# h3jia/bayesfast

Measured on AMD Instinct MI355X. Metric: leapfrog steps/sec (all chains), 4096 chains x 64-d quadratic surrogate, higher is better.
Workload: dtype f64

## Files before the change

bayesfast_amd/_lib.py:

```python
import ctypes as C
import os
import subprocess

_HERE = os.path.dirname(os.path.abspath(__file__))
LIB_PATH = os.environ.get('BFHIP_LIBRARY') or os.path.join(_HERE, 'libbfhip.so')
CSRC = os.path.join(_HERE, 'csrc')

SC_FIELDS = ('log_step', 'log_bar', 'hbar', 'mu', 'count', 'fg_n', 'bg_n', 'n_samples', 'prev_update',
             'adapt_window', 'i_iter', 'error')
SC_N = len(SC_FIELDS)
VEC_FIELDS = ('q', 'var', 'fg_mean', 'fg_raw', 'bg_mean', 'bg_raw')
VEC_N = len(VEC_FIELDS)
MAT_N = 6
STAT_STRIDE = 11
NSTATS = ('logp', 'energy', 'tree_depth', 'tree_size', 'mean_tree_accept', 'step_size', 'step_size_bar',
          'warmup', 'energy_change', 'max_energy_change', 'diverging')
HSTATS = ('logp', 'energy', 'n_int_step', 'accept_stat', 'accepted', 'step_size', 'step_size_bar', 'warmup',
          'energy_change', 'diverging')
MAX_DIM = 128
MAX_TREEDEPTH = 12
TREE_MODE_WORK = 4162
LAG_EDGES = tuple((j + 1) if j < 2 else ((1 << ((j + 1) // 2)) if (j & 1) else (3 << (j // 2 - 1))) for j in range(64))

_dp = C.POINTER(C.c_double)
# ... 49 lines not shown
    'bfhip_ctx_destroy': (None, [_vp]),
    'bfhip_ctx_set_stream': (C.c_int, [_vp, _vp]),
    'bfhip_ctx_synchronize': (C.c_int, [_vp]),
    'bfhip_density_upload': (C.c_int, [_vp, C.POINTER(DensityDesc)]),
    'bfhip_logp_grad': (C.c_int, [_vp, C.c_int, _vp, C.c_int, _vp, _vp]),
    'bfhip_constraint': (C.c_int, [_vp, C.c_int, C.c_int, _vp, _vp, _vp]),
    'bfhip_leapfrog': (C.c_int, [_vp, C.c_int] + [_vp] * 8),
    'bfhip_sampler_run': (C.c_int, [_vp, C.POINTER(SamplerConfig), C.c_int, C.c_int, _vp, _vp, _vp, C.c_int,
                                    C.c_int, _vp, _vp, _vp]),
    'bfhip_tnuts_run': (C.c_int, [_vp, C.POINTER(SamplerConfig), C.POINTER(Tempering), C.c_int, C.c_int, _vp, _vp, _vp, _vp,
                                  C.c_int, C.c_int, _vp, _vp, _vp, _vp]),
    'bfhip_rng_seed': (C.c_int, [_vp, C.c_int, C.c_uint64, C.c_uint64, _vp]),
    'bfhip_chain_init': (C.c_int, [_vp, C.c_int, C.c_int, _vp, C.c_double, _vp, _vp, C.c_double, C.c_int, _vp, _vp]),
    'bfhip_metric_init_full': (C.c_int, [_vp, C.c_int, C.c_int, _vp, C.c_double, _vp, _vp]),
    'bfhip_polymodel_upload': (C.c_int, [_vp, C.POINTER(PolymodelDesc)]),
    'bfhip_polymodel_eval': (C.c_int, [_vp, C.c_int, _vp, _vp, _vp]),
    'bfhip_chi2_stage': (C.c_int, [_vp, C.c_int, C.c_int, C.c_int, _vp, _vp, _vp, _vp, _vp, C.c_double, _vp, _vp]),
    'bfhip_pipeline_upload': (C.c_int, [_vp, C.POINTER(PipelineDesc)]),
    'bfhip_design_block': (C.c_int, [_vp, C.c_int, C.c_int, C.c_int, _vp, _vp, _vp, C.c_int, C.c_int]),
    'bfhip_gram': (C.c_int, [_vp, C.c_int, C.c_int, C.c_int, _vp, C.c_int, _vp, _vp, _vp]),
    'bfhip_tree_size_mode_share': (C.c_int, [_vp, C.c_int, C.c_int, _vp, C.c_int, C.c_int, C.c_double, _vp]),
    'bfhip_solve_spd': (C.c_int, [_vp, C.c_int, C.c_int, _vp, _vp, _vp]),
    'bfhip_lstsq': (C.c_int, [_vp, C.c_int, C.c_int, C.c_int, _vp, C.c_int, _vp, _vp, _vp, C.c_int, _vp, _vp]),
    'bfhip_sort_keys': (C.c_int, [_vp, C.c_long, _vp, _vp, _vp]),
    'bfhip_order_keys': (C.c_int, [_vp, C.c_long, _vp, _vp]),
    'bfhip_count_keys': (C.c_int, [_vp, C.c_long, _vp, C.c_long, _vp, C.c_int, _vp]),
    'bfhip_importance_weights': (C.c_int, [_vp, C.c_long, _vp, _vp, C.c_double, _vp, _vp]),
    'bfhip_polar_ns': (C.c_int, [_vp, C.c_int, _vp, _vp, C.c_int, _vp, _vp]),
    'bfhip_ndtri': (C.c_int, [_vp, C.c_long, _vp, _vp]),
    'bfhip_ica_tanh': (C.c_int, [_vp, C.c_long, C.c_long, C.c_int, _vp, _vp]),
    'bfhip_ica_assemble': (C.c_int, [_vp, C.c_int, C.c_int, _vp, C.c_long, C.c_long, _vp, _vp, _vp, _vp]),
    'bfhip_ica_post': (C.c_int, [_vp, C.c_int, _vp, _vp, _vp, C.c_int, C.c_int, _vp, _vp]),
    'bfhip_spline_build': (C.c_int, [_vp, C.c_int, C.c_long, _vp, _vp, _vp, _vp, C.c_int, _vp, C.c_int, C.c_int, _vp, C.c_double,
                                     C.c_int, C.c_int, C.c_int, _vp, _vp, _vp, _vp]),
    'bfhip_kde_cdf': (C.c_int, [_vp, C.c_int, C.c_long, _vp, _vp, _vp, C.c_int, _vp, _vp]),
    'bfhip_spline_apply': (C.c_int, [_vp, C.c_int, C.c_long, C.c_int, _vp, _vp, _vp, _vp, _vp, _vp]),
    'bfhip_bridge_sums': (C.c_int, [_vp, C.c_long, _vp, C.c_long, _vp, C.c_double, _vp]),
    'bfhip_bridge_terms': (C.c_int, [_vp, C.c_long, _vp, _vp, C.c_long, _vp, _vp, C.c_double, _vp, _vp]),
    'bfhip_logmeanexp_stats': (C.c_int, [_vp, C.c_long, _vp, _vp, _vp, _vp]),
    'bfhip_acor_moments': (C.c_int, [_vp, C.c_int, C.c_long, C.c_int, C.c_long, _vp, _vp, _vp]),
    'bfhip_acor_lag_sums': (C.c_int, [_vp, C.c_int, C.c_long, C.c_int, C.c_long, _vp, _vp, _vp, C.c_long, C.c_int, _vp, _vp]),
    'bfhip_diag_columns': (C.c_int, [_vp, C.c_int, C.c_long, C.c_long, C.c_long, _vp, C.c_int, C.c_long, C.c_int, C.c_int, C.c_int, _vp,
                                     _vp]),
    'bfhip_diag_extent': (C.c_int, [_vp, C.c_int, C.c_long, _vp, _vp, _vp]),
    'bfhip_diag_sort': (C.c_int, [_vp, C.c_long, _vp, C.c_int, _vp, _vp]),
    'bfhip_diag_rank': (C.c_int, [_vp, C.c_long, _vp, _vp, C.c_int, _vp]),
    'bfhip_logp_hess': (C.c_int, [_vp, C.c_int, _vp, C.c_int, _vp, _vp, _vp]),
    'bfhip_laplace_opt': (C.c_int, [_vp, C.POINTER(LaplaceOpts), C.c_int, _vp, _vp, _vp, _vp, _vp]),
    'bfhip_pipeline_logp_hess': (C.c_int, [_vp, C.c_int, _vp, C.c_int, C.c_int, _vp, _vp, _vp]),
    'bfhip_pipeline_laplace_opt': (C.c_int, [_vp, C.POINTER(LaplaceOpts), C.c_int, C.c_int, _vp, _vp, _vp, _vp, _vp]),
    'bfhip_wave_sum_probe': (C.c_int, [_vp, C.c_int, C.c_int, C.c_int, _vp, _vp]),
}
HESS_FULL, HESS_GAUSS_NEWTON = 0, 1
WSUM_MAX = 7
WSUM_FORMS = {'built': 0, 'packed': 1, 'unpacked': 2}
ACOR_MAX_GROUPS = 256
DIAG_BATCH = 16

_lib = None


def build(verbose=False):
    out = None if verbose else subprocess.DEVNULL
    subprocess.check_call(['make', '-C', CSRC, '-j4'], stdout=out)
    return LIB_PATH


def lib():
    global _lib
    if _lib is None:
        if not os.path.exists(LIB_PATH):
            raise RuntimeError(
                'bayesfast_amd: the HIP extension %s is missing; build it with '
                '`python -c "import __graft_entry__ as g; g.build()"` or `make -C bayesfast_amd/csrc`. '
                'There is no CPU fallback.' % LIB_PATH)
        import torch
        L = C.CDLL(LIB_PATH)
        for name, (res, args) in SYMBOLS.items():
            f = getattr(L, name)
            f.restype = res
            f.argtypes = args
        _lib = L
    return _lib


class BfhipError(RuntimeError):
    pass


def debug_set(key, value):
    f = lib().bfhip_debug_set
    f.restype, f.argtypes = C.c_int, [C.c_char_p, C.c_longlong]
    check(f(key.encode(), int(value)))


def debug_get(key):
    f = lib().bfhip_debug_get
    f.restype, f.argtypes = C.c_longlong, [C.c_char_p]
    return int(f(key.encode()))


def debug_buffer(key, tensor_or_none):
    f = lib().bfhip_debug_buffer
    f.restype, f.argtypes = C.c_int, [C.c_char_p, C.c_void_p]
    check(f(key.encode(), None if tensor_or_none is None else C.c_void_p(tensor_or_none.data_ptr())))


# ... 12 lines not shown
```

bayesfast_amd/csrc/bfhip_lone.h:

```cpp

#pragma push_macro("exp")
#pragma push_macro("log")
#pragma push_macro("sqrt")
#pragma push_macro("sincospi")
#undef exp
#undef log
#undef sqrt
#undef sincospi
__device__ inline double ln_opq(double x) { asm("" : "+v"(x)); return x; }
#define LN_EXPV(x) ln_opq(exp(ln_opq(x)))
#define LN_LOGV(x) ln_opq(log(ln_opq(x)))
#define LN_SQRTV(x) ln_opq(sqrt(ln_opq(x)))
#define LN_EXP(x) rfl(LN_EXPV(x))
#define LN_LOG(x) rfl(LN_LOGV(x))
#define LN_SQRT(x) rfl(LN_SQRTV(x))

enum { LN_CONT = 0, LN_NEW = 1, LN_DONE = 2 };
enum { LF_NONE = 0, LF_LEAF = 1, LF_INIT = 2 };
enum { LV_CMD = 0, LV_CLOSE, LV_EO, LV_EVAL, LV_DIR, LV_INIT, LV_N = 8 };

template <int W, int DEC>
struct LoneGeo {
    using PG = PipeGeo<W, DEC>;
    static constexpr int DP = 16 * W, NS = 4 * W, NMAT = PG::NMAT, KS = PG::KS, KPJ = PG::KPJ;
// ... 375 lines not shown
            WF[2 * DP + lane] = load_vec(BFHIP_VEC_BG_MEAN, 0.); WF[3 * DP + lane] = load_vec(BFHIP_VEC_BG_RAW, 0.);
        }
        if (lane < 5) WF[4 * DP + lane] = scp[BFHIP_SC_FG_N + lane];
    }
    if (i_iter < a.iter_end && err == 0) {
        draw_momentum();
        eps = (i_iter < nw) ? step_now : step_bar;
        draw_dir();
        post_new(1);
        fly = LF_INIT;
    } else {
        if (lane == 0) VI[LV_CMD] = LN_DONE;
        kdone = true;
    }

    for (;;) {
        LTRACE(1, 0);
        __syncthreads();
        LTRACE(1, 1);
        if (kdone) break;
        kb = 0;
        bool ended = false;
        if (prev == LF_INIT) {
            q = lfv(0); p = lfv(1); g = lfv(2);
            const double E0 = rfl(LF[3 * DP]), logp0 = rfl(LF[3 * DP + 1]);
            KBAR(); KBAR();
            if (!init_tree(E0, logp0)) { kdone = true; }
        } else if (prev == LF_LEAF) {
            {
                const double lq_ = lfv(0), lp_ = lfv(1), lg_ = lfv(2);
                const double le_ = LF[3 * DP], ll_ = LF[3 * DP + 1];
                TPq = lq_; TRp = lp_; TPg = lg_;
                E_pend = rfl(le_);
                lp_pend = rfl(ll_);
            }
            LTRACE(1, 4);
            int unit = U_EVAL, lev = 0;
            nlf += 1;
            n_prop += 1;
            double dE = E_pend - start_energy;
            if (dE != dE) dE = INFINITY;
            if (fabs(dE) > fabs(max_de)) max_de = dE;
            T_E = E_pend;
            T_logp = lp_pend;
            T_acc = 0.;
            if (!(fabs(dE) < a.cfg.max_change)) {
                diverged = 1;
                unit = U_ABORT;
            }
            LTRACE(1, 11);
            KBAR();
            LTRACE(1, 10);
            double aw = -dE - w_off;
            const double e_aw = LN_EXPV(aw);
            const double ps0 = L0p + TRp;
            double r2[2] = {ps0 * (var * L0p), ps0 * (var * TRp)};
            wave_sum_n<2>(r2);
            if (unit == U_EVAL) {
                T_W = rfl(e_aw);
                if (aw > 600.) {
                    const double sc_ = LN_EXP(-aw);
                    tree_W = tree_W * sc_;
                    if (lane == 0)
                        for (int l2 = 0; l2 < depth; ++l2) LS[l2 * LS_N + LS_LS] *= sc_;
                    L0_W *= sc_;
                    w_off = w_off + aw;
                    aw = 0.;
                    T_W = 1.;
                }
                const double pacc = (w_off == 0.) ? T_W : LN_EXP(-dE);
                T_acc = pacc > 1. ? 1. : pacc;
                TLp = TRp;
                TPs = TRp;
                unit = U_MERGE;
            }
            LTRACE(1, 5);
            if (unit == U_MERGE && (i_leaf & 1) && depth > 0) {
                T_acc = L0_acc + T_acc;
                const double Wsum = L0_W + T_W;
                if (Wsum != Wsum) err = 2;
                const double u = bf_u01(bf_xoshiro_next(rs));
                lev = 1;
                if ((r2[0] <= 0.) || (r2[1] <= 0.)) {
                    unit = U_ABORT;
                } else {
                    if (!((u * Wsum < T_W) || (u == 0.))) {
                        TPq = L0q;
                        TPg = L0g;
                        T_E = rfl(LS[LS_E]);
                        T_logp = rfl(LS[LS_LOGP]);
                    }
                    T_W = Wsum;
                    TPs = L0p + TRp;
                    TLp = L0p;
                }
            }
            LTRACE(1, 6);
            KBAR();
            LTRACE(1, 7);
            while (unit == U_MERGE && lev < depth && ((i_leaf >> lev) & 1)) {
                const int slot = SL_STACK + 4 * lev;
                const double A = ldv(slot + 0), B = ldv(slot + 1), S1 = ldv(slot + 2);
                const double psum = S1 + TPs;
                const double vA = var * A, vB = var * B, vC = var * TLp, vD = var * TRp;
                const double ps1 = S1 + TLp;
                const double ps2 = B + TPs;
                double r6[6] = {psum * vA, psum * vD, ps1 * vA, ps1 * vC, ps2 * vB, ps2 * vD};
                wave_sum_n<6>(r6);
                const bool turning = (r6[0] <= 0.) || (r6[1] <= 0.) || (r6[2] <= 0.) || (r6[3] <= 0.) || (r6[4] <= 0.) || (r6[5] <= 0.);
                const double *lsp = LS + lev * LS_N;
                T_acc = rfl(lsp[LS_ACC]) + T_acc;
                const double Wsum = rfl(lsp[LS_LS]) + T_W;
                if (Wsum != Wsum) err = 2;
                const double u = bf_u01(bf_xoshiro_next(rs));
                const bool keep_t2 = (u * Wsum < T_W) || (u == 0.);
                lev += 1;
                if (turning) {
                    unit = U_ABORT;
                } else {
                    if (!keep_t2) {
                        TPq = ldv(slot + 3);
                        TPg = ldv(SL_PG + lev - 1);
                        T_E = rfl(lsp[LS_E]);
                        T_logp = rfl(lsp[LS_LOGP]);
                    }
                    T_W = Wsum;
                    TLp = A;
                    TPs = psum;
                }
            }
            if (unit == U_MERGE) {
                if (lev < depth) {
                    if (lev == 0) {
                        L0p = TRp;
                        L0q = TPq;
                        L0g = TPg;
                        L0_W = T_W;
                        L0_acc = T_acc;
                    } else {
                        const int slot = SL_STACK + 4 * lev;
                        stv(slot + 0, TLp); stv(slot + 1, TRp); stv(slot + 2, TPs); stv(slot + 3, TPq);
                        stv(SL_PG + lev, TPg);
                    }
                    if (lane == 0) {
                        double *lsp = LS + lev * LS_N;
                        lsp[LS_LS] = T_W; lsp[LS_ACC] = T_acc;
                        lsp[LS_E] = (lev == 0) ? E_pend : T_E;
                        lsp[LS_LOGP] = (lev == 0) ? lp_pend : T_logp;
                    }
                    i_leaf += 1;
                    unit = U_DONE;
                } else {
                    unit = U_DBL_END;
                }
            }
            LTRACE(1, 8);
            if (unit == U_ABORT) {
                for (int al = (diverged ? 0 : lev); al < depth; ++al)
                    if ((i_leaf >> al) & 1) T_acc = rfl(LS[al * LS_N + LS_ACC]) + T_acc;
                depth += 1;
                acc_sum += T_acc;
                unit = U_END1;
            } else if (unit == U_DBL_END) {
                double ps = ldv(SL_PSUM);
                const double oldL = ldv(SL_LEFT_P), oldR = ldv(SL_RIGHT_P);
                depth += 1;
                acc_sum += T_acc;
                {
                    if (T_W != T_W || tree_W != tree_W) err = 2;
                    const double u = bf_u01(bf_xoshiro_next(rs));
                    if ((u * tree_W < T_W) || (u == 0.)) {
                        stv(SL_PROP_Q, TPq);
                        stv(SL_PROPG, TPg);
                        prop_E = T_E;
                        prop_logp = T_logp;
                    }
                    tree_W = tree_W + T_W;
                }
                ps += TPs;
                const double vN = var * TRp, vT = var * TLp, vL = var * oldL, vR = var * oldR;
                double r6[6];
                if (dir > 0) {
                    const double ps1 = ps + TLp, ps2 = oldR + TPs;
// ... 182 lines not shown
```

bayesfast_amd/csrc/bfhip_nuts_pipe.h:

```cpp


enum { SL_PROPG = SL_STACK + 4 * BFHIP_MAX_TREEDEPTH, SL_PG = SL_PROPG + 1, SL_PIPE_N = SL_PG + BFHIP_MAX_TREEDEPTH };

template <int W, int DEC = 0>
struct PipeGeo {
    static constexpr int NMAT = DEC == 1 ? 3 : 2;
    static constexpr int KS = DEC == 1 ? (W == 2 ? 2 : 1) : ((W == 2 || W == 4) ? 2 : 1);
    static constexpr int KPJ = (4 * W) / KS, NJOB = NMAT * W * KS, NTL = 12;
    static constexpr int MPS = KPJ > 8 ? 2 : 1;
    static_assert(NJOB <= 16 && KPJ <= 8 * MPS, "one job per wave, eight MFMA sites");
    static constexpr size_t lds_doubles() {
        using G = SamplerGeo<W>;
        return (size_t)NMAT * G::NS * G::XS + (size_t)16 * BFHIP_MAX_TREEDEPTH * LS_N + 4 + (size_t)16 * CS_N +
               (size_t)16 * NTL * G::DP + (size_t)NMAT * KS * 16 * G::GS;
    }
};

template <int QUAD> struct PipeAcc { typedef d4_t type; };
template <> struct PipeAcc<1> { typedef double type; };
template <> struct PipeAcc<2> { typedef d2_t type; };
__device__ inline d4_t bf_pipe_mfma(double a_, double b_, d4_t c_) { return __builtin_amdgcn_mfma_f64_16x16x4f64(a_, b_, c_, 0, 0, 0); }
__device__ inline double bf_pipe_mfma(double a_, double b_, double c_) { return __builtin_amdgcn_mfma_f64_4x4x4f64(a_, b_, c_, 0, 0, 0); }

template <int W, bool TR, int DEC = 0, int QUAD = 0>
__global__ __launch_bounds__(1024) void bf_nuts_pipe_kernel(DevModel m, SamplerArgs a) {
    using G = SamplerGeo<W>;
    using PG = PipeGeo<W, DEC>;
    constexpr int DP = G::DP, NS = G::NS, XS = G::XS, GS = G::GS;
    constexpr int KS_P = PG::KS, KPJ_P = PG::KPJ, NJOB_P = PG::NJOB, NTL = PG::NTL, NMAT = PG::NMAT, MPS = PG::MPS;
    constexpr int MAXL = BFHIP_MAX_TREEDEPTH;
    static_assert(DP <= 64, "one dimension per lane");
    extern __shared__ __attribute__((aligned(16))) double lds[];
    double *XB = lds;
    double *LS = XB + NMAT * NS * XS;
    int *alive = (int *)(LS + 16 * MAXL * LS_N);
    double *CS = LS + 16 * MAXL * LS_N + 4;
    double *TB = CS + 16 * CS_N;
    double *GB = TB + 16 * NTL * DP;

    const int tid = threadIdx.x, lane = tid & 63;
    const int w = __builtin_amdgcn_readfirstlane(tid >> 6);
    int cpg = a.cpg > 0 ? a.cpg : 16;
    int chain = blockIdx.x * cpg + w;
    bool real = w < cpg && chain < a.n_chain;
    if (a.tail_list) {
        const int cnt = rfl(a.tail_count[0]);
        cpg = cnt <= a.n_cu ? 1 : (cnt <= 2 * a.n_cu ? 2 : 4);
        const int idx = blockIdx.x * cpg + w;
        real = w < cpg && idx < cnt;
        chain = real ? rfl(a.tail_list[idx]) : 0;
    }
    const int d = m.d;
    const bool lane_ok = lane < DP;

    double afr[KPJ_P];
    {
        const int slot_m = w / (W * KS_P), rem = w % (W * KS_P), t = rem / KS_P, kp = rem % KS_P;
        const double *Af = (slot_m == 0 ? m.Sf : (slot_m == 1 ? m.Hf : m.Hdf)) + (t * NS + kp * KPJ_P) * 64 + lane;
#pragma unroll
        for (int s = 0; s < KPJ_P; ++s) afr[s] = (w < NJOB_P) ? Af[s * 64] : 0.;
    }
    if (tid < 8) alive[tid] = 0;
    const double c_lin = lane_ok ? m.pd[PD_LIN * DP + lane] : 0.;
    const double c_mu = lane_ok ? m.pd[PD_MU * DP + lane] : 0.;
    const double c_dmu = (DEC == 1 && lane_ok) ? m.pd[PD_DMU * DP + lane] : 0.;
    const double c_smu = lane_ok ? m.pd[PD_SMU * DP + lane] : 0.;
    const int c_kind = (TR && lane_ok) ? (int)m.pd[PD_KIND * DP + lane] : 0;
    const double c_lo = (TR && lane_ok) ? m.pd[PD_LO * DP + lane] : 0., c_rg = (TR && lane_ok) ? m.pd[PD_RG * DP + lane] : 1.;
    double xs = 0., jac = 1., gj = 0., logdet_l = 0.;

    double q = 0., p = 0., g = 0., var = 1.;
    double TLp = 0., TPs = 0., TPq = 0.;
    double TRp = 0.;
    double L0p = 0., L0q = 0.;
    double TPg = 0., L0g = 0.;
    uint64_t rs[4] = {0, 0, 0, 0};
    int i_iter = 0, mode = M_DONE, err = 0;
    double eps = 0., eps_t = 0.;
    int dir = 1, depth = 0, i_leaf = 0, n_prop = 0, diverged = 0;
    double start_energy = 0., acc_sum = 0.;
    double T_W = 0., T_acc = 0.;
    double max_de = 0., w_off = 0., L0_W = 0., L0_acc = 0.;
    bool pend = false;
// ... 242 lines not shown
                const int xi = (lane >> 2) * XS + w + 16 * (lane & 3);
                XB[xi] = xs;
                XB[NS * XS + xi] = xs - c_mu;
                if constexpr (DEC == 1) XB[2 * NS * XS + xi] = xs - c_dmu;
            }
        }
        if (lane == 0) {
            if (mode != M_DONE) alive[trip & 1] = 1;
            if (evaluating) atomicOr((unsigned *)&alive[2 + (trip & 1)], 1u << w);
        }
        TRACE(1);
        __syncthreads();
        TRACE(2);
        if (rfl(alive[trip & 1]) == 0) break;
        const unsigned ev_mask = (unsigned)rfl(alive[2 + (trip & 1)]);
        if (tid == 0) { alive[(trip + 1) & 1] = 0; alive[2 + ((trip + 1) & 1)] = 0; alive[4 + ((trip + 1) & 1)] = 0; }

        const bool job = ev_mask != 0 && w < NJOB_P;
        typename PipeAcc<QUAD>::type acc = {};
        const double *Xf = XB + ((w / (W * KS_P)) * NS + (w % KS_P) * KPJ_P) * XS + (QUAD ? (lane & ~15) + (lane & 3) : lane);
        double x_pre[MPS], x_pr2[QUAD == 2 ? MPS : 1];
#pragma unroll
        for (int u = 0; u < MPS; ++u) x_pre[u] = job ? Xf[u * XS] : 0.;
        if constexpr (QUAD == 2) {
#pragma unroll
            for (int u = 0; u < MPS; ++u) x_pr2[u] = job ? Xf[u * XS + 4] : 0.;
        }
#define BF_MF(K)                                                                                            \
        do {                                                                                                \
            if ((K) * MPS < KPJ_P) {                                                                        \
                double x_cur[MPS], x_cu2[QUAD == 2 ? MPS : 1];                                             \
                _Pragma("unroll") for (int u = 0; u < MPS; ++u) x_cur[u] = x_pre[u];                        \
                if constexpr (QUAD == 2) { _Pragma("unroll") for (int u = 0; u < MPS; ++u) x_cu2[u] = x_pr2[u]; } \
                if (((K) + 1) * MPS < KPJ_P && job) {                                                       \
                    _Pragma("unroll") for (int u = 0; u < MPS; ++u) x_pre[u] = Xf[((((K) + 1) * MPS < KPJ_P ? ((K) + 1) * MPS : 0) + u) * XS]; \
                    if constexpr (QUAD == 2) { _Pragma("unroll") for (int u = 0; u < MPS; ++u) x_pr2[u] = Xf[((((K) + 1) * MPS < KPJ_P ? ((K) + 1) * MPS : 0) + u) * XS + 4]; } \
                }                                                                                           \
                _Pragma("unroll") for (int u = 0; u < MPS; ++u) {                                           \
                    asm volatile("" : "+v"(acc) : : "memory");                                              \
                    if constexpr (QUAD == 2) {                                                              \
                        if (job) {                                                                          \
                            acc[0] = bf_pipe_mfma(afr[((K) * MPS < KPJ_P ? (K) * MPS : 0) + u], x_cur[u], acc[0]); \
                            acc[1] = bf_pipe_mfma(afr[((K) * MPS < KPJ_P ? (K) * MPS : 0) + u], x_cu2[u], acc[1]); \
                        }                                                                                   \
                    } else {                                                                                \
                        if (job) acc = bf_pipe_mfma(afr[((K) * MPS < KPJ_P ? (K) * MPS : 0) + u], x_cur[u], acc); \
                    }                                                                                       \
                    asm volatile("" : "+v"(acc) : : "memory");                                              \
                }                                                                                           \
            }                                                                                               \
        } while (0)
        int unit = pend ? U_EVAL : U_DONE, lev = 0;
        bool ended = false;
        pend = false;
        BF_MF(0);
        TRACE(3);
        double dE = 0.;
        if (unit == U_EVAL) {
            nlf += 1;
            n_prop += 1;
            dE = E_pend - start_energy;
            if (dE != dE) dE = INFINITY;
            if (fabs(dE) > fabs(max_de)) max_de = dE;
            cs_set(CS_T_E, E_pend);
            cs_set(CS_T_LOGP, lp_pend);
            T_acc = 0.;
            if (!(fabs(dE) < a.cfg.max_change)) {
                diverged = 1;
                unit = U_ABORT;
            }
        }
        BF_MF(1);
        if (unit == U_EVAL) {
            double aw = -dE - w_off;
            if (aw > 600.) {
                const double sc_ = uexp(-aw);
                cs_set(CS_TREE_W, cs_get(CS_TREE_W) * sc_);
                if (lane == 0)
                    for (int l2 = 0; l2 < depth; ++l2) lsw[l2 * LS_N + LS_LS] *= sc_;
                L0_W *= sc_;
                w_off = w_off + aw;
                aw = 0.;
            }
            T_W = uexp(aw);
            const double pacc = (w_off == 0.) ? T_W : uexp(-dE);
            T_acc = pacc > 1. ? 1. : pacc;
            TLp = TRp;
            TPs = TRp;
            unit = U_MERGE;
        }
        BF_MF(2);
        TRACE(9);
        if (unit == U_MERGE && (i_leaf & 1) && depth > 0) {
            const double ps0 = L0p + TRp;
            double r2[2] = {ps0 * (var * L0p), ps0 * (var * TRp)};
            wave_sum_n<2>(r2);
            T_acc = L0_acc + T_acc;
            const double Wsum = L0_W + T_W;
            if (Wsum != Wsum) err = 2;
            const double u = bf_u01(bf_xoshiro_next(rs));
            lev = 1;
            if ((r2[0] <= 0.) || (r2[1] <= 0.)) {
                unit = U_ABORT;
            } else {
                if (!((u * Wsum < T_W) || (u == 0.))) {
                    TPq = L0q;
                    TPg = L0g;
                    cs_set(CS_T_E, rfl(lsw[LS_E]));
                    cs_set(CS_T_LOGP, rfl(lsw[LS_LOGP]));
                }
                T_W = Wsum;
                TPs = L0p + TRp;
                TLp = L0p;
            }
        }
        BF_MF(3);
        while (unit == U_MERGE && lev < depth && ((i_leaf >> lev) & 1)) {
            const int slot = SL_STACK + 4 * lev;
            const double A = ldv(slot + 0), B = ldv(slot + 1), S1 = ldv(slot + 2);
            const double psum = S1 + TPs;
            const double vA = var * A, vB = var * B, vC = var * TLp, vD = var * TRp;
            const double ps1 = S1 + TLp;
            const double ps2 = B + TPs;
            double r6[6] = {psum * vA, psum * vD, ps1 * vA, ps1 * vC, ps2 * vB, ps2 * vD};
            wave_sum_n<6>(r6);
            const bool turning = (r6[0] <= 0.) || (r6[1] <= 0.) || (r6[2] <= 0.) || (r6[3] <= 0.) || (r6[4] <= 0.) || (r6[5] <= 0.);
            const double *lsp = lsw + lev * LS_N;
            T_acc = rfl(lsp[LS_ACC]) + T_acc;
            const double Wsum = rfl(lsp[LS_LS]) + T_W;
            if (Wsum != Wsum) err = 2;
            const double u = bf_u01(bf_xoshiro_next(rs));
            const bool keep_t2 = (u * Wsum < T_W) || (u == 0.);
            lev += 1;
            if (turning) {
                unit = U_ABORT;
            } else {
                if (!keep_t2) {
                    TPq = ldv(slot + 3);
                    TPg = ldv(SL_PG + lev - 1);
                    cs_set(CS_T_E, rfl(lsp[LS_E]));
                    cs_set(CS_T_LOGP, rfl(lsp[LS_LOGP]));
                }
                T_W = Wsum;
                TLp = A;
                TPs = psum;
            }
        }
        BF_MF(4);
        TRACE(10);
        if (unit == U_MERGE) {
            if (lev < depth) {
                if (lev == 0) {
                    L0p = TRp;
                    L0q = TPq;
                    L0g = TPg;
                    L0_W = T_W;
                    L0_acc = T_acc;
                } else {
                    const int slot = SL_STACK + 4 * lev;
                    stv(slot + 0, TLp); stv(slot + 1, TRp); stv(slot + 2, TPs); stv(slot + 3, TPq);
                    stv(SL_PG + lev, TPg);
                }
                if (lane == 0) {
                    double *lsp = lsw + lev * LS_N;
                    lsp[LS_LS] = T_W; lsp[LS_ACC] = T_acc;
                    lsp[LS_E] = (lev == 0) ? E_pend : cs_get(CS_T_E);
                    lsp[LS_LOGP] = (lev == 0) ? lp_pend : cs_get(CS_T_LOGP);
                }
                i_leaf += 1;
                unit = U_DONE;
            } else {
                unit = U_DBL_END;
            }
        }
        BF_MF(5);
        if (__builtin_expect(unit == U_ABORT, 0)) {
            for (int al = (diverged ? 0 : lev); al < depth; ++al)
                if ((i_leaf >> al) & 1) T_acc = rfl(lsw[al * LS_N + LS_ACC]) + T_acc;
            depth += 1;
            acc_sum += T_acc;
            unit = U_END1;
        } else if (unit == U_DBL_END) {
            double ps = ldv(SL_PSUM);
            const double oldL = ldv(SL_LEFT_P), oldR = ldv(SL_RIGHT_P);
            depth += 1;
            acc_sum += T_acc;
            {
                const double tree_W = cs_get(CS_TREE_W);
                if (T_W != T_W || tree_W != tree_W) err = 2;
                const double u = bf_u01(bf_xoshiro_next(rs));
                if ((u * tree_W < T_W) || (u == 0.)) {
                    stv(SL_PROP_Q, TPq);
                    stv(SL_PROPG, TPg);
                    cs_set(CS_PROP_E, cs_get(CS_T_E));
                    cs_set(CS_PROP_LOGP, cs_get(CS_T_LOGP));
                }
                cs_set(CS_TREE_W, tree_W + T_W);
            }
            ps += TPs;
            const double vN = var * TRp, vT = var * TLp, vL = var * oldL, vR = var * oldR;
// ... 156 lines not shown
```

bayesfast_amd/csrc/bfhip_sampler.hip:

```cpp
#include <type_traits>
#include <cstring>
#include <cstdio>
#include <cstdlib>
#include "bfhip_eval.h"
#include "bfhip_metric.h"
#include "bfhip_pld.h"
#include "bfhip_oob.h"

__device__ __attribute__((noinline)) static double bf_exp_ni(double x) { return exp(x); }
__device__ __attribute__((noinline)) static double bf_log_ni(double x) { return log(x); }
__device__ __attribute__((noinline)) static double bf_sqrt_ni(double x) { return sqrt(x); }
__device__ __attribute__((noinline)) static void bf_sincospi_ni(double x, double *s, double *c) { sincospi(x, s, c); }
#define exp(x) bf_exp_ni(x)
#define log(x) bf_log_ni(x)
#define sqrt(x) bf_sqrt_ni(x)
#define sincospi(x, s, c) bf_sincospi_ni(x, s, c)
#define uexp(x) rfl(bf_exp_ni(x))
#define ulog(x) rfl(bf_log_ni(x))
#define usqrt(x) rfl(bf_sqrt_ni(x))

#include "bfhip_sampler_defs.h"

#include "bfhip_wave.h"

// ... 1518 lines not shown
#pragma unroll
                for (int e = 0; e < E; ++e) kin += p[e] * (var[e] * p[e]);
            }
            kin = kin_ready ? kin_fast : wave_sum(kin);
            E_new = 0.5 * kin - logp_new;
        }

        stamp(3);
        TRACE(9);
        const int mode_in = mode;
        if constexpr (CHAIN_UNITS) {
            bool first = true;
            do {
                run_unit(first && unit_in == U_EVAL && have_eval, E_new, logp_new);
                first = false;
            } while (unit != U_EVAL && unit != U_DONE);
        } else
        if (unit_in == U_EVAL) run_unit(have_eval, E_new, logp_new);
        else run_unit(false, 0., 0.);
        TRACE(10);
        stamp(unit_in == U_EVAL ? (mode_in == M_INIT ? 4 : 5) : (unit_in == U_MERGE_RUN ? 6 : (unit_in == U_DBL_END ? 7 : (unit_in == U_DONE ? 9 : 8))));
    }

#ifdef BF_TRACE
    if (a.stamps && w == 0 && blockIdx.x == 0)
        for (int i = lane; i < BF_TRACE * 16; i += 64) a.stamps[i] = TRC[i];
#endif
    if constexpr (STAMPS) {
        if (a.stamps && lane == 0)
            for (int k = 0; k < 10; ++k) {
                a.stamps[((size_t)blockIdx.x * 16 + w) * 20 + k] = st_acc[k];
                a.stamps[((size_t)blockIdx.x * 16 + w) * 20 + 10 + k] = st_cnt[k];
            }
    }
    if (real) {
        store_vec(BFHIP_VEC_Q, q);
        if (lane == 0) {
            for (int k = 0; k < 4; ++k) a.rng[(size_t)chain * 4 + k] = rs[k];
            scp[BFHIP_SC_LOG_STEP] = cs_get(CS_LOG_STEP);
            scp[BFHIP_SC_LOG_BAR] = cs_get(CS_LOG_BAR);
            scp[BFHIP_SC_HBAR] = cs_get(CS_HBAR);
            scp[BFHIP_SC_COUNT] = cs_get(CS_COUNT);
            scp[BFHIP_SC_I_ITER] = (double)i_iter;
            scp[BFHIP_SC_ERROR] = (double)err;
            if (a.n_leapfrog && nlf) atomicAdd(a.n_leapfrog, nlf);
        }
    }
}

#ifdef BF_TRACE
#undef TRACE
#define TRACE(k) do { if (w == 0 && blockIdx.x == 0 && trip_no < BF_TRACE && lane == 0) TRC[trip_no * 16 + (k)] = clock64(); } while (0)
#endif
#include "bfhip_nuts_pipe.h"
#include "bfhip_lone.h"

static bool sampler_plain(const DevModel &m) { return bf_model_plain(m) && !bf_tune().no_plain; }

static int sampler_ksplit(const DevModel &m) {
    const int W = m.DP / 16;
    const int n_mat = (m.has_quad ? 1 : 0) + (m.use_bound ? 1 : 0) + (m.use_decay ? 1 : 0);
    int ks = 1;
    while (2 * ks <= W && n_mat * W * 2 * ks <= 16) ks *= 2;
    return ks;
}
static int sampler_gb_slots(const DevModel &m) {
    const int n_mat = (m.has_quad ? 1 : 0) + (m.use_bound ? 1 : 0) + (m.use_decay ? 1 : 0);
    return n_mat * sampler_ksplit(m) > 1 ? n_mat * sampler_ksplit(m) : 1;
}

static size_t sampler_lds_base(const DevModel &m, bool plain) {
    const int W = m.DP / 16, DP = m.DP, NS = 4 * W;
    size_t dbl = (size_t)3 * NS * 65 + (size_t)sampler_gb_slots(m) * 16 * (DP + 1) + (size_t)16 * BFHIP_MAX_TREEDEPTH * LS_N + 4 +
                 (size_t)16 * CS_N + (size_t)PD_N * DP;
    if (DP <= 64 && plain)
        dbl += (size_t)2 * DP * (DP + 2) + (size_t)2 * 16 * DP;
    else if (DP <= 64)
        dbl += (size_t)DP * DP * ((m.has_quad ? 1 : 0) + (m.use_bound ? 1 : 0) + (m.use_decay ? 1 : 0));
    return dbl;
}
static size_t sampler_cubic_doubles(const DevModel &m) {
    return (size_t)2 * m.n2 * m.n2 + (size_t)((m.n3 + 15) >> 4) * m.n3 * m.n3 * 16 + 2;
}
static bool sampler_cubic_lds(const DevModel &m, bool plain) {
    return m.has_cubic && m.n2 <= 64 && m.n3 <= 64 &&
           (sampler_lds_base(m, plain) + sampler_cubic_doubles(m)) * sizeof(double) <= BF_LDS_MAX;
}
static size_t sampler_lds_bytes(const DevModel &m, bool plain, int nwv = 16) {
    if (m.pld.on && m.pld.stream)
        return (((sampler_lds_base(m, false) + 1) & ~(size_t)1) + pld_s_lds_doubles(m.DP, m.pld.MP, m.pld.KC)) * sizeof(double);
    if (m.pld.on)
        return (((sampler_lds_base(m, false) + 1) & ~(size_t)1) +
                pld_lds_doubles(m.DP, m.pld.MP, m.pld.PP, m.pld.KS2, m.pld.n_ent, nwv == 8 ? PLD_XS8 : PLD_XS)) * sizeof(double);
    return (sampler_lds_base(m, plain) + (sampler_cubic_lds(m, plain) ? sampler_cubic_doubles(m) : 0)) * sizeof(double);
}
size_t bf_sampler_lds_bytes_base(const DevModel &m) { return ((sampler_lds_base(m, false) + 1) & ~(size_t)1) * sizeof(double); }

static int wave_layout_cpg(const bfhip_ctx *ctx, int n_chain, int nwv) {
    const int forced = bf_tune().wave_cpg;
    if (forced > 0) return forced < nwv ? forced : nwv;
    int cpg = nwv;
    while (cpg > 1 && (n_chain + cpg / 2 - 1) / (cpg / 2) <= ctx->n_cu) cpg /= 2;
    return cpg;
}

template <int W, bool NUTS, bool STAMPS, int FS, int FULLM = 0>
// ... 425 lines not shown
```

bayesfast_amd/csrc/bfhip_wave_probe.hip:

```cpp
#include "bfhip_common.h"
#include "bfhip_wave.h"

template <int N>
__global__ __launch_bounds__(64) void bf_wave_sum_probe_kernel(int form, const double *__restrict__ in, double *__restrict__ out) {
    const int lane = threadIdx.x;
    const size_t base = (size_t)blockIdx.x * N;
    double v[N];
#pragma unroll
    for (int i = 0; i < N; ++i) v[i] = in[(base + i) * 64 + lane];
    if (form == BFHIP_WSUM_PACKED) wave_sum_n_packed<N>(v);
    else if (form == BFHIP_WSUM_UNPACKED) wave_sum_n_unpacked<N>(v);
    else wave_sum_n<N>(v);
    if (lane == 0) {
#pragma unroll
        for (int i = 0; i < N; ++i) out[base + i] = v[i];
    }
}

template <int N>
static void wave_sum_probe_launch(bfhip_ctx *ctx, int n_batch, int form, const double *in, double *out) {
    hipLaunchKernelGGL(bf_wave_sum_probe_kernel<N>, dim3((unsigned)n_batch), dim3(64), 0, ctx->stream, form, in, out);
}

extern "C" int bfhip_wave_sum_probe(bfhip_ctx *ctx, int n_batch, int n_val, int form, const double *in, double *out) {
    BfDeviceGuard dev_guard(ctx);
    if (!ctx || n_batch < 0 || n_val < 1 || n_val > BFHIP_WSUM_MAX || form < BFHIP_WSUM_BUILT || form > BFHIP_WSUM_UNPACKED ||
        (n_batch > 0 && (!in || !out)))
        return bf_set_error(BFHIP_ERR_ARG, "bfhip_wave_sum_probe: invalid argument");
    if (n_batch == 0) return 0;
    switch (n_val) {
        case 1: wave_sum_probe_launch<1>(ctx, n_batch, form, in, out); break;
        case 2: wave_sum_probe_launch<2>(ctx, n_batch, form, in, out); break;
        case 3: wave_sum_probe_launch<3>(ctx, n_batch, form, in, out); break;
        case 4: wave_sum_probe_launch<4>(ctx, n_batch, form, in, out); break;
        case 5: wave_sum_probe_launch<5>(ctx, n_batch, form, in, out); break;
        case 6: wave_sum_probe_launch<6>(ctx, n_batch, form, in, out); break;
        default: wave_sum_probe_launch<7>(ctx, n_batch, form, in, out); break;
    }
    BF_HIP_CHECK(hipGetLastError());
    return 0;
}
```

include/bfhip.h:

```cpp
#ifndef BFHIP_H
#define BFHIP_H
#include <stddef.h>
#include <stdint.h>

#ifdef __cplusplus
extern "C" {
#endif

typedef struct bfhip_ctx bfhip_ctx;

#define BFHIP_OK 0
#define BFHIP_ERR_ARG (-1)
#define BFHIP_ERR_STATE (-2)
#define BFHIP_ERR_HIP (-3)
#define BFHIP_ERR_UNSUPPORTED (-4)

#define BFHIP_MAX_DIM 128
#define BFHIP_MAX_TREEDEPTH 12

int bfhip_version(void);
const char *bfhip_last_error(void);

int bfhip_ctx_create(bfhip_ctx **out, int device, void *stream);
void bfhip_ctx_destroy(bfhip_ctx *ctx);
// ... 185 lines not shown
int bfhip_spline_build(bfhip_ctx *ctx, int d, long n, const double *sorted, const double *data, const double *w, const double *h,
                       int n_grid, const double *grid, int edge_bins, int n_inner, const double *inner, double max_width, int split,
                       int max_add, int stride, double *out_x, double *out_y, double *out_c, int *out_n);

int bfhip_spline_apply(bfhip_ctx *ctx, int mode, long n, int d, const double *x, const int *knot_off, const double *knots,
                       const double *values, const double *coef, double *out);

int bfhip_bridge_sums(bfhip_ctx *ctx, long n_a, const double *a, long n_b, const double *b, double logr, double *out2);

int bfhip_bridge_terms(bfhip_ctx *ctx, long n_p, const double *logp_p, const double *logq_p, long n_q, const double *logp_q,
                       const double *logq_q, double logr, double *f1, double *f2);

int bfhip_logmeanexp_stats(bfhip_ctx *ctx, long n, const double *x, const double *y, double *out3, double *terms);

int bfhip_ica_tanh(bfhip_ctx *ctx, long n, long n_pad, int d, double *y, double *partial);
int bfhip_ica_assemble(bfhip_ctx *ctx, int d, int nb, const double *p, long n, long n_pad, const double *partial, const double *w,
                       double *a, double *meas_k);
int bfhip_ica_post(bfhip_ctx *ctx, int d, const double *w1, double *w, const double *resid, int k, int n_meas, double *wbuf,
                   double *meas);

int bfhip_polar_ns(bfhip_ctx *ctx, int d, const double *a, double *x, int n_iter, double *work, double *resid);

int bfhip_acor_moments(bfhip_ctx *ctx, int n_w, long n_t, int n_d, long ldw, const double *x, double *mean, double *inv);
int bfhip_acor_lag_sums(bfhip_ctx *ctx, int n_w, long n_t, int n_d, long ldw, const double *x, const double *mean, const double *inv,
                        long t0, int n_lag, double *work, double *out);

#define BFHIP_DIAG_BATCH 16
#define BFHIP_DIAG_PLAIN 0
#define BFHIP_DIAG_FOLD 1
#define BFHIP_DIAG_BELOW 2
int bfhip_diag_columns(bfhip_ctx *ctx, int n_chain, long h, long ldw, long ldr, const void *x, int is_f32, long since, int k0, int nb,
                       int mode, const double *c, double *out);
int bfhip_diag_extent(bfhip_ctx *ctx, int n_series, long h, const double *series, double *lo, double *hi);
int bfhip_diag_sort(bfhip_ctx *ctx, long n, const double *series, int b, uint64_t *keys_sorted, uint32_t *order);
int bfhip_diag_rank(bfhip_ctx *ctx, long n, const uint64_t *keys_sorted, const uint32_t *order, int b, double *z);

int bfhip_logp_hess(bfhip_ctx *ctx, int n, const double *x, int original_space, double *logp, double *grad, double *hess);

typedef struct {
    int max_iter;
    double xtol;
} bfhip_laplace_opts;

int bfhip_laplace_opt(bfhip_ctx *ctx, const bfhip_laplace_opts *opts, int n_start, const double *x0, double *x, double *logp,
                      double *hess, double *info);

#define BFHIP_HESS_FULL 0
#define BFHIP_HESS_GAUSS_NEWTON 1
int bfhip_pipeline_logp_hess(bfhip_ctx *ctx, int n, const double *x, int original_space, int hess_kind, double *logp, double *grad,
                             double *hess);
int bfhip_pipeline_laplace_opt(bfhip_ctx *ctx, const bfhip_laplace_opts *opts, int hess_kind, int n_start, const double *x0, double *x,
                               double *logp, double *hess, double *info);

#define BFHIP_WSUM_MAX 7
#define BFHIP_WSUM_BUILT 0
#define BFHIP_WSUM_PACKED 1
#define BFHIP_WSUM_UNPACKED 2
int bfhip_wave_sum_probe(bfhip_ctx *ctx, int n_batch, int n_val, int form, const double *in, double *out);


#ifdef __cplusplus
}
#endif
#endif
```

Baseline: 717.8 million.

## Batch NUTS subtree merge U-turn checks across levels into one wave reduction

Replaces the per-level sequential merge loop, which ran one wave-wide reduction per tree level, with a batched merge. Stack entries for up to NB levels are loaded together, all six U-turn dot products per level are computed at once, and they are reduced in a single wave_sum, with optional fusion into the leaf's first reduction. This targets the serialized cross-lane reduction latency when several levels close at the same time. In exchange it does speculative work on levels past an early U-turn and uses more registers. The wave-sum probe is also extended to cover up to 20 values.

```diff
diff --git a/bayesfast_amd/_lib.py b/bayesfast_amd/_lib.py
--- a/bayesfast_amd/_lib.py
+++ b/bayesfast_amd/_lib.py
@@ -125,7 +125,7 @@
     'bfhip_wave_sum_probe': (C.c_int, [_vp, C.c_int, C.c_int, C.c_int, _vp, _vp]),
 }
 HESS_FULL, HESS_GAUSS_NEWTON = 0, 1
-WSUM_MAX = 7
+WSUM_MAX = 20
 WSUM_FORMS = {'built': 0, 'packed': 1, 'unpacked': 2}
 ACOR_MAX_GROUPS = 256
 DIAG_BATCH = 16
diff --git a/bayesfast_amd/csrc/bfhip_lone.h b/bayesfast_amd/csrc/bfhip_lone.h
--- a/bayesfast_amd/csrc/bfhip_lone.h
+++ b/bayesfast_amd/csrc/bfhip_lone.h
@@ -451,10 +451,30 @@
             KBAR();
             LTRACE(1, 10);
             double aw = -dE - w_off;
+            const double ps0 = L0p + TRp;
+#ifdef BF_MERGE_SEQUENTIAL
             const double e_aw = LN_EXPV(aw);
-            const double ps0 = L0p + TRp;
             double r2[2] = {ps0 * (var * L0p), ps0 * (var * TRp)};
             wave_sum_n<2>(r2);
+#else
+            constexpr int NB_UP = BF_MERGE_NB_LONE;
+            const int n_up = (unit == U_EVAL) ? bf_merge_upper_levels(i_leaf, depth) : 0;
+            BfMergeLv<NB_UP> mlv;
+            double mps[NB_UP], r2[2 + 6 * NB_UP];
+            double e_aw;
+            if (n_up > 0) {
+                bf_merge_load<NB_UP>(ldv, 1, n_up, mlv);
+                e_aw = LN_EXPV(aw);
+                r2[0] = ps0 * (var * L0p); r2[1] = ps0 * (var * TRp);
+                bf_merge_products<NB_UP, 2>(mlv, var, L0p, ps0, TRp, r2, mps);
+                wave_sum_n<2 + 6 * NB_UP>(r2);
+            } else {
+                e_aw = LN_EXPV(aw);
+                double r0[2] = {ps0 * (var * L0p), ps0 * (var * TRp)};
+                wave_sum_n<2>(r0);
+                r2[0] = r0[0]; r2[1] = r0[1];
+            }
+#endif
             if (unit == U_EVAL) {
                 T_W = rfl(e_aw);
                 if (aw > 600.) {
@@ -497,6 +517,7 @@
             LTRACE(1, 6);
             KBAR();
             LTRACE(1, 7);
+#ifdef BF_MERGE_SEQUENTIAL
             while (unit == U_MERGE && lev < depth && ((i_leaf >> lev) & 1)) {
                 const int slot = SL_STACK + 4 * lev;
                 const double A = ldv(slot + 0), B = ldv(slot + 1), S1 = ldv(slot + 2);
@@ -528,6 +549,16 @@
                     TPs = psum;
                 }
             }
+#else
+            if (unit == U_MERGE && n_up > 0) {
+                auto ls_get = [&](int l, int f) -> double { return rfl(LS[l * LS_N + f]); };
+                auto set_te = [&](double e_, double lp_) { T_E = e_; T_logp = lp_; };
+                const int np = n_up < NB_UP ? n_up : NB_UP;
+                bf_merge_walk<NB_UP, 2>(mlv, mps, r2, np, ldv, ls_get, set_te, SL_PG, rs, unit, lev, err, T_acc, T_W, TLp, TPs, TPq, TPg);
+                bf_merge_close<NB_UP>(mlv, false, n_up - np, var, TRp, ldv, ls_get, set_te, SL_PG, rs, unit, lev, err, T_acc, T_W, TLp, TPs,
+                                      TPq, TPg);
+            }
+#endif
             if (unit == U_MERGE) {
                 if (lev < depth) {
                     if (lev == 0) {
diff --git a/bayesfast_amd/csrc/bfhip_merge.h b/bayesfast_amd/csrc/bfhip_merge.h
--- /dev/null
+++ b/bayesfast_amd/csrc/bfhip_merge.h
@@ -0,0 +1,111 @@
+#pragma once
+
+#ifndef BF_MERGE_NB_PIPE
+#define BF_MERGE_NB_PIPE 2
+#endif
+#ifndef BF_MERGE_NB_LONE
+#define BF_MERGE_NB_LONE 2
+#endif
+#ifndef BF_MERGE_LOAD_AT
+#define BF_MERGE_LOAD_AT 2
+#endif
+
+template <int NB>
+struct BfMergeLv { double A[NB], B[NB], S1[NB]; };
+
+__device__ __forceinline__ int bf_merge_upper_levels(int i_leaf, int depth) {
+    if (!(i_leaf & 1) || depth < 1) return 0;
+    const int t = __builtin_ctz(~(unsigned)i_leaf);
+    return (t < depth ? t : depth) - 1;
+}
+
+template <int NB, class LDV>
+__device__ __forceinline__ void bf_merge_load(LDV &&ldv, int lev0, int n, BfMergeLv<NB> &m) {
+#pragma unroll
+    for (int k = 0; k < NB; ++k) {
+        if (k == 0 || k < n) {
+            const int slot = SL_STACK + 4 * (lev0 + k);
+            m.A[k] = ldv(slot + 0); m.B[k] = ldv(slot + 1); m.S1[k] = ldv(slot + 2);
+        } else {
+            m.A[k] = m.A[0]; m.B[k] = m.B[0]; m.S1[k] = m.S1[0];
+        }
+    }
+}
+
+template <int NB, int OFF, int NR>
+__device__ __forceinline__ void bf_merge_products(const BfMergeLv<NB> &m, double var, double TLp, double TPs, double TRp, double (&r)[NR],
+                                         double (&ps)[NB]) {
+    static_assert(OFF + 6 * NB <= NR, "the pass's products fit the reduction");
+    const double vD = var * TRp;
+#pragma unroll
+    for (int k = 0; k < NB; ++k) {
+        const double A = m.A[k], B = m.B[k], S1 = m.S1[k];
+        const double psum = S1 + TPs;
+        const double vA = var * A, vB = var * B, vC = var * TLp;
+        const double ps1 = S1 + TLp;
+        const double ps2 = B + TPs;
+        r[OFF + 6 * k + 0] = psum * vA; r[OFF + 6 * k + 1] = psum * vD; r[OFF + 6 * k + 2] = ps1 * vA;
+        r[OFF + 6 * k + 3] = ps1 * vC; r[OFF + 6 * k + 4] = ps2 * vB; r[OFF + 6 * k + 5] = ps2 * vD;
+        ps[k] = psum;
+        TLp = A;
+        TPs = psum;
+    }
+}
+
+template <int NB, int OFF, int NR, class LDV, class LSG, class SETE>
+__device__ __forceinline__ void bf_merge_walk(const BfMergeLv<NB> &m, const double (&ps)[NB], const double (&r)[NR], int n, LDV &&ldv, LSG &&ls,
+                                     SETE &&set_te, int sl_pg, uint64_t (&rs)[4], int &unit, int &lev, int &err, double &T_acc, double &T_W,
+                                     double &TLp, double &TPs, double &TPq, double &TPg) {
+    const int lev0 = lev;
+    int merged = 0, sib = -1;
+#pragma unroll
+    for (int k = 0; k < NB; ++k) {
+        if (k < n && unit == U_MERGE) {
+            const bool turning = (r[OFF + 6 * k + 0] <= 0.) || (r[OFF + 6 * k + 1] <= 0.) || (r[OFF + 6 * k + 2] <= 0.) ||
+                                 (r[OFF + 6 * k + 3] <= 0.) || (r[OFF + 6 * k + 4] <= 0.) || (r[OFF + 6 * k + 5] <= 0.);
+            T_acc = ls(lev, LS_ACC) + T_acc;
+            const double Wsum = ls(lev, LS_LS) + T_W;
+            if (Wsum != Wsum) err = 2;
+            const double u = bf_u01(bf_xoshiro_next(rs));
+            const bool keep_t2 = (u * Wsum < T_W) || (u == 0.);
+            lev += 1;
+            if (turning) {
+                unit = U_ABORT;
+            } else {
+                if (!keep_t2) sib = k;
+                T_W = Wsum;
+                merged = k + 1;
+            }
+        }
+    }
+    if (merged > 0) {
+        double A = m.A[0], S = ps[0];
+#pragma unroll
+        for (int k = 1; k < NB; ++k)
+            if (merged > k) { A = m.A[k]; S = ps[k]; }
+        TLp = A;
+        TPs = S;
+    }
+    if (sib >= 0) {
+        const int sl = lev0 + sib;
+        TPq = ldv(SL_STACK + 4 * sl + 3);
+        TPg = ldv(sl_pg + sl);
+        set_te(ls(sl, LS_E), ls(sl, LS_LOGP));
+    }
+}
+
+template <int NB, class LDV, class LSG, class SETE>
+__device__ __forceinline__ void bf_merge_close(BfMergeLv<NB> &m, bool first, int n, double var, double TRp, LDV &&ldv, LSG &&ls, SETE &&set_te,
+                                      int sl_pg, uint64_t (&rs)[4], int &unit, int &lev, int &err, double &T_acc, double &T_W,
+                                      double &TLp, double &TPs, double &TPq, double &TPg) {
+    while (n > 0 && unit == U_MERGE) {
+        const int np = n < NB ? n : NB;
+        if (!first) bf_merge_load<NB>(ldv, lev, np, m);
+        first = false;
+        double r[6 * NB], ps[NB];
+        bf_merge_products<NB, 0>(m, var, TLp, TPs, TRp, r, ps);
+        wave_sum_n<6 * NB>(r);
+        bf_merge_walk<NB, 0>(m, ps, r, np, ldv, ls, set_te, sl_pg, rs, unit, lev, err, T_acc, T_W, TLp, TPs, TPq, TPg);
+        n -= np;
+    }
+}
diff --git a/bayesfast_amd/csrc/bfhip_nuts_pipe.h b/bayesfast_amd/csrc/bfhip_nuts_pipe.h
--- a/bayesfast_amd/csrc/bfhip_nuts_pipe.h
+++ b/bayesfast_amd/csrc/bfhip_nuts_pipe.h
@@ -29,6 +29,7 @@
     constexpr int DP = G::DP, NS = G::NS, XS = G::XS, GS = G::GS;
     constexpr int KS_P = PG::KS, KPJ_P = PG::KPJ, NJOB_P = PG::NJOB, NTL = PG::NTL, NMAT = PG::NMAT, MPS = PG::MPS;
     constexpr int MAXL = BFHIP_MAX_TREEDEPTH;
+    constexpr int NB_UP = BF_MERGE_NB_PIPE;
     static_assert(DP <= 64, "one dimension per lane");
     extern __shared__ __attribute__((aligned(16))) double lds[];
     double *XB = lds;
@@ -377,6 +378,11 @@
         } while (0)
         int unit = pend ? U_EVAL : U_DONE, lev = 0;
         bool ended = false;
+#ifndef BF_MERGE_SEQUENTIAL
+        BfMergeLv<NB_UP> mlv;
+        const int n_up = pend ? bf_merge_upper_levels(i_leaf, depth) : 0;
+        if (BF_MERGE_LOAD_AT == 0 && n_up > 0) bf_merge_load<NB_UP>(ldv, 1, n_up, mlv);
+#endif
         pend = false;
         BF_MF(0);
         TRACE(3);
@@ -416,6 +422,9 @@
         }
         BF_MF(2);
         TRACE(9);
+#ifndef BF_MERGE_SEQUENTIAL
+        if (BF_MERGE_LOAD_AT == 1 && unit == U_MERGE && n_up > 0) bf_merge_load<NB_UP>(ldv, 1, n_up, mlv);
+#endif
         if (unit == U_MERGE && (i_leaf & 1) && depth > 0) {
             const double ps0 = L0p + TRp;
             double r2[2] = {ps0 * (var * L0p), ps0 * (var * TRp)};
@@ -440,6 +449,7 @@
             }
         }
         BF_MF(3);
+#ifdef BF_MERGE_SEQUENTIAL
         while (unit == U_MERGE && lev < depth && ((i_leaf >> lev) & 1)) {
             const int slot = SL_STACK + 4 * lev;
             const double A = ldv(slot + 0), B = ldv(slot + 1), S1 = ldv(slot + 2);
@@ -471,6 +481,12 @@
                 TPs = psum;
             }
         }
+#else
+        if (unit == U_MERGE && n_up > 0)
+            bf_merge_close<NB_UP>(mlv, BF_MERGE_LOAD_AT < 2, n_up, var, TRp, ldv, [&](int l, int f) -> double { return rfl(lsw[l * LS_N + f]); },
+                                  [&](double e_, double lp_) { cs_set(CS_T_E, e_); cs_set(CS_T_LOGP, lp_); }, SL_PG, rs, unit, lev, err,
+                                  T_acc, T_W, TLp, TPs, TPq, TPg);
+#endif
         BF_MF(4);
         TRACE(10);
         if (unit == U_MERGE) {
diff --git a/bayesfast_amd/csrc/bfhip_sampler.hip b/bayesfast_amd/csrc/bfhip_sampler.hip
--- a/bayesfast_amd/csrc/bfhip_sampler.hip
+++ b/bayesfast_amd/csrc/bfhip_sampler.hip
@@ -1594,6 +1594,7 @@
 #undef TRACE
 #define TRACE(k) do { if (w == 0 && blockIdx.x == 0 && trip_no < BF_TRACE && lane == 0) TRC[trip_no * 16 + (k)] = clock64(); } while (0)
 #endif
+#include "bfhip_merge.h"
 #include "bfhip_nuts_pipe.h"
 #include "bfhip_lone.h"
 
diff --git a/bayesfast_amd/csrc/bfhip_wave_probe.hip b/bayesfast_amd/csrc/bfhip_wave_probe.hip
--- a/bayesfast_amd/csrc/bfhip_wave_probe.hip
+++ b/bayesfast_amd/csrc/bfhip_wave_probe.hip
@@ -28,6 +28,7 @@
         (n_batch > 0 && (!in || !out)))
         return bf_set_error(BFHIP_ERR_ARG, "bfhip_wave_sum_probe: invalid argument");
     if (n_batch == 0) return 0;
+    static_assert(BFHIP_WSUM_MAX == 20, "one case per number of values");
     switch (n_val) {
         case 1: wave_sum_probe_launch<1>(ctx, n_batch, form, in, out); break;
         case 2: wave_sum_probe_launch<2>(ctx, n_batch, form, in, out); break;
@@ -35,7 +36,20 @@
         case 4: wave_sum_probe_launch<4>(ctx, n_batch, form, in, out); break;
         case 5: wave_sum_probe_launch<5>(ctx, n_batch, form, in, out); break;
         case 6: wave_sum_probe_launch<6>(ctx, n_batch, form, in, out); break;
-        default: wave_sum_probe_launch<7>(ctx, n_batch, form, in, out); break;
+        case 7: wave_sum_probe_launch<7>(ctx, n_batch, form, in, out); break;
+        case 8: wave_sum_probe_launch<8>(ctx, n_batch, form, in, out); break;
+        case 9: wave_sum_probe_launch<9>(ctx, n_batch, form, in, out); break;
+        case 10: wave_sum_probe_launch<10>(ctx, n_batch, form, in, out); break;
+        case 11: wave_sum_probe_launch<11>(ctx, n_batch, form, in, out); break;
+        case 12: wave_sum_probe_launch<12>(ctx, n_batch, form, in, out); break;
+        case 13: wave_sum_probe_launch<13>(ctx, n_batch, form, in, out); break;
+        case 14: wave_sum_probe_launch<14>(ctx, n_batch, form, in, out); break;
+        case 15: wave_sum_probe_launch<15>(ctx, n_batch, form, in, out); break;
+        case 16: wave_sum_probe_launch<16>(ctx, n_batch, form, in, out); break;
+        case 17: wave_sum_probe_launch<17>(ctx, n_batch, form, in, out); break;
+        case 18: wave_sum_probe_launch<18>(ctx, n_batch, form, in, out); break;
+        case 19: wave_sum_probe_launch<19>(ctx, n_batch, form, in, out); break;
+        default: wave_sum_probe_launch<20>(ctx, n_batch, form, in, out); break;
     }
     BF_HIP_CHECK(hipGetLastError());
     return 0;
diff --git a/include/bfhip.h b/include/bfhip.h
--- a/include/bfhip.h
+++ b/include/bfhip.h
@@ -261,7 +261,7 @@
 int bfhip_pipeline_laplace_opt(bfhip_ctx *ctx, const bfhip_laplace_opts *opts, int hess_kind, int n_start, const double *x0, double *x,
                                double *logp, double *hess, double *info);
 
-#define BFHIP_WSUM_MAX 7
+#define BFHIP_WSUM_MAX 20
 #define BFHIP_WSUM_BUILT 0
 #define BFHIP_WSUM_PACKED 1
 #define BFHIP_WSUM_UNPACKED 2
```

Measured after the change: 645.9 million. 0.9x the previous value.
